# vwxyzjn/cleanrl

Measured on NVIDIA H100. Metric: env steps/sec (SPS) PPO Breakout num_envs=1024, higher is better.
Workload: dtype bf16

## Files before the change

### cleanrl_b200/csrc/net_tc.cu

```cuda
#include <cuda.h>
#include <algorithm>
#include "tc_base.cuh"
#include "tc_conv_win.cuh"
#include "tc_conv23.cuh"
#include "tc_conv1_u8.cuh"
#include "tc_gemm_tma.cuh"
#include "tc_wgrad_win.cuh"
#include "tc_reduce.cuh"
#include "tc_aux.cuh"
#include "tc_heads.cuh"
#include "tc_heads_wide.cuh"
#include "tc_lstm.cuh"

namespace b200rl {

struct NatureLayout {
    int A;
    int64_t c1w, c1b, c2w, c2b, c3w, c3b, fcw, fcb, hw, hb, total;
    int64_t w1f, w2f, w2dg, w3f, w3dg, wfcf, wfcdg, w1l, w1sc, packed_total;
    bool wide; int G; int64_t whf, whdg, hbp;
    int64_t wih, whh, bih, bhh, whhp;
    explicit NatureLayout(int A_) : A(A_), wih(-1), whh(-1), bih(-1), bhh(-1), whhp(-1) {
        int64_t o = 0;
        c1w = o; o += 32 * 4 * 8 * 8;  c1b = o; o += 32;
// ... 83 lines not shown
    p.A = x; p.M = n; p.nchunks = nchunks;
}


static void win_defaults(WinParams& p) { memset(&p, 0, sizeof(p)); p.scale = 1.f; }
static int round8(int v) { return (v + 7) & ~7; }
static void win_conv1(WinParams& p, const bf16* x0, const int64_t* rows, int64_t n) {
    p.A = x0; p.rows = rows; p.n = (int)n; p.G = 441; p.Wp = 21; p.M = n * 441;
    p.tpi_shift = 2;
    p.n_images = rows ? (int64_t)1 << 24 : n;
    p.ntaps = 4; p.shift[0] = 0; p.shift[1] = 1; p.shift[2] = 21; p.shift[3] = 22; p.WR = round8(128 + 22);
}
static void wgw_defaults(WGradWinParams& w) { memset(&w, 0, sizeof(w)); }

static const int kC1Ctas = 264, kC2Ctas = 132, kC3Ctas = 132;
static WPlan conv1_wgrad_plan(int64_t n, bool u8) {
    return u8 ? wgrad_plan(n * 512, kC2Ctas, 512) : wgrad_plan(n * 512, kC1Ctas, 128);
}
static WPlan conv2_wgrad_plan(int64_t n) { return wgrad_plan(n * 100, kC2Ctas, 128); }
static WPlan conv3_wgrad_plan(int64_t n) { return wgrad_plan(n * 81, kC3Ctas, 128); }

static size_t wgrad_win_bytes(int splits, int nslots) { return (size_t)splits * nslots * 64 * 64 * sizeof(float); }
static size_t wgrad_win_bias_bytes(int splits) { return (size_t)splits * 64 * sizeof(float); }
static int launch_wgrad_win(const WGradWinParams& p, int ctas, cudaStream_t s, const char* what) {
    const size_t smem = (size_t)kWgradWinStages * ((size_t)p.WRX * 128 * p.cpr + 128 * 128) + 4096 + 1024;
    static SmemAttrCache attr;
    if (int rc0 = attr.ensure(tc_wgrad_win, smem, what)) return rc0;
    CUtensorMap tmX, tmY;
    memset(&tmX, 0, sizeof(tmX)); memset(&tmY, 0, sizeof(tmY));
    const int use_tma = p.tpi_shift ? 0 : 1;
    if (p.rows_per_cta % 128 != 0) return fail(B200RL_ERR_INVALID_ARGUMENT, "%s: rows per CTA must be a multiple of 128", what);
    if (ctas < 1 || (int64_t)(ctas - 1) * p.rows_per_cta >= p.M)
        return fail(B200RL_ERR_INVALID_ARGUMENT, "%s: every row split must own at least one row", what);
    int rc;
    if (use_tma) {
        if (p.rows || p.ldy != 64 || p.ncolsY != 64)
            return fail(B200RL_ERR_INVALID_ARGUMENT, "%s: linear-grid mode needs contiguous rows and 64-channel dY", what);
        if ((rc = make_tmap_2d(&tmX, p.X, p.M, (int64_t)p.cpr * 64, p.WRX, what))) return rc;
        if ((rc = make_tmap_2d(&tmY, p.Y, p.M, 64, 128, what))) return rc;
    } else {
        if ((128 << p.tpi_shift) < p.G) return fail(B200RL_ERR_INVALID_ARGUMENT, "%s: steps per image too small", what);
        if ((rc = make_tmap_3d(&tmX, p.X, p.n_images, p.G, (int64_t)p.cpr * 64, p.WRX, what))) return rc;
    }
    const dim3 grid((unsigned)ceil_div(p.nslots / 2, kWgradWinTilesPerCta), ctas);
    tc_wgrad_win<<<grid, kWgradWinThreads, smem, s>>>(tmX, tmY, p, use_tma);
    return check_launch(what);
}

}

using namespace b200rl;

namespace b200rl {
static bool head_ok(int A) { return A >= 1 && A < kMaxWideHeads; }
static size_t wide_dhead_bytes(int64_t n, const NatureLayout& L) { return ((size_t)n * L.G * 2 + 255) & ~(size_t)255; }
static size_t wide_small_bytes(int64_t n, const NatureLayout& L, int A1) {
    return wide_dhead_bytes(n, L) + colsum_f32_ws(n, A1);
}

static int trunk_fwd(const NatureLayout& L, const NatureActs& Q, const float* params, const bf16* P, bf16* act, int64_t n,
                     cudaStream_t s) {
    int rc;
    KGemmParams p;
    Conv23Params cp;
    cp.n = (int)n; cp.b2 = params + L.c2b; cp.b3 = params + L.c3b; cp.act2 = act + Q.act2; cp.act3 = act + Q.act3;
    cp.m2 = reinterpret_cast<uint32_t*>(act + Q.m2); cp.m3 = reinterpret_cast<uint32_t*>(act + Q.m3);
    { ProfScope ps(s, "conv23_fwd", 2.0 * n * 81 * 64 * 512 + 2.0 * n * 49 * 64 * 576,
                   (double)n * (12800 * 2 + 5184 * 2 + 648 + 3136 * 2 + 392));
// ... 8 lines not shown
}

static int trunk_bwd(const NatureLayout& L, const NatureActs& Q, const bf16* P, bf16* act, float* grads, int64_t n,
                     float* wsbig, float* wssmall, void* tail_ready_event, bool dact1_fused, cudaStream_t s) {
    int rc;
    KGemmParams p;
    {
        int splits;
        { ProfScope ps(s, "fc_wgrad", 2.0 * n * 512 * 3136, (double)n * (3136 + 512) * 2 + 512.0 * 3136 * 4);
          if ((splits = launch_wgrad_tma(act + Q.dhid, 512, act + Q.act3, 3136, n, wsbig, s, "naturecnn/fc_wgrad")) < 0) return splits; }
        { ProfScope ps(s, "wgrad_fold_bias", 0, 0);
          note_launches(1); tc_fold_fc<<<(unsigned)ceil_div((int64_t)512 * 3136, 256), 256, 0, s>>>(wsbig, splits, 512, 13 * 256, 512, 3136, 64, 49, 1.f, grads + L.fcw);
          if ((rc = colsum(act + Q.dhid, n, 512, 512, wssmall, grads + L.fcb, s))) return rc; }
        if (tail_ready_event) {
            cudaError_t e = cudaEventRecord(reinterpret_cast<cudaEvent_t>(tail_ready_event), s);
            if (e != cudaSuccess) return fail(B200RL_ERR_CUDA, "naturecnn_backward: cudaEventRecord: %s", cudaGetErrorString(e));
        }
        gemm_rowmajor(p, act + Q.dhid, n, 8);
        p.Bw = P + L.wfcdg; p.N = 3136; p.out = act + Q.dact3a; p.out2 = act + Q.dact3b; p.dual_dact3 = 1;
        p.ldo = 3136; p.mask_bits = reinterpret_cast<const uint32_t*>(act + Q.m3);
        { ProfScope ps(s, "fc_dgrad", 2.0 * n * 512 * 3136, (double)n * ((3136 + 512) * 2 + 392) + 512.0 * 3136 * 2);
          if ((rc = launch_gemm_tma<128, 3>(p, s, "naturecnn/fc_dgrad"))) return rc; }
    }
    WGradWinParams gw;
    WinParams wp;
    FoldWin fw;
    {
        wgw_defaults(gw);
        gw.X = act + Q.act2; gw.M = n * 81; gw.n = (int)n; gw.G = 81; gw.cpr = 1; gw.nslots = 10; gw.WRX = round8(128 + 20);
        for (int t = 0; t < 9; ++t) gw.shift[t] = (t / 3) * 9 + (t % 3);
        const int st[10] = {0, 1, 2, 3, 4, 5, 6, 7, 7, 8};
        for (int k = 0; k < 10; ++k) { gw.slot_tap[k] = st[k]; gw.slot_cc[k] = 0; }
        gw.Y = act + Q.dact3a; gw.ldy = 64; gw.ncolsY = 64;
        const WPlan pl = conv3_wgrad_plan(n);
        gw.rows_per_cta = pl.rows_per_cta; gw.ws = wsbig; gw.wsb = wssmall;
        { ProfScope ps(s, "conv3_wgrad", 2.0 * n * 49 * 64 * 576, (double)n * (5184 + 5184) * 2);
          if ((rc = launch_wgrad_win(gw, pl.splits, s, "naturecnn/conv3_wgrad"))) return rc; }
        memset(&fw, 0, sizeof(fw));
        fw.layer = 3; fw.S = pl.splits; fw.nslots = 10; fw.Cout = 64; fw.scale = 1.f; fw.bscale = 1.f;
        for (int k = 0; k < 10; ++k) { fw.slot_tap[k] = st[k]; fw.slot_skip[k] = (k == 8); }
        { ProfScope ps(s, "wgrad_fold_bias", 0, 0);
          fw.wsb = wssmall; fw.db = grads + L.c3b;
          tc_fold_win<<<(unsigned)ceil_div(640 * 64 + 64, 32), 256, 0, s>>>(wsbig, fw, grads + L.c3w);
          if ((rc = check_launch("naturecnn/conv3_fold"))) return rc; }
        win_defaults(wp);
        wp.A = act + Q.dact3b; wp.n = (int)n; wp.G = 121; wp.Wp = 11; wp.M = n * 121; wp.ntaps = 9;
        for (int ky = 0; ky < 3; ++ky) for (int kx = 0; kx < 3; ++kx) wp.shift[ky * 3 + kx] = (2 - ky) * 11 + (2 - kx);
        wp.WR = round8(128 + 24);
        wp.Bw = P + L.w3dg; wp.N = 64; wp.vH = 9; wp.vW = 9; wp.out_mode = WOUT_DACT2;
        wp.out = act + Q.dact2a; wp.out2 = act + Q.dact2b; wp.mask_bits = reinterpret_cast<const uint32_t*>(act + Q.m2);
        { ProfScope ps(s, "conv3_dgrad", 2.0 * n * 81 * 64 * 576, (double)n * ((7744 + 6400 + 7744) * 2 + 648));
          if ((rc = launch_conv_win_t<128, 1, 4, 9>(wp, s, "naturecnn/conv3_dgrad"))) return rc; }
    }
    {
        wgw_defaults(gw);
        gw.X = act + Q.act1; gw.M = n * 100; gw.n = (int)n; gw.G = 100; gw.cpr = 2; gw.nslots = 8; gw.WRX = round8(128 + 11);
        gw.shift[0] = 0; gw.shift[1] = 1; gw.shift[2] = 10; gw.shift[3] = 11;
        for (int k = 0; k < 8; ++k) { gw.slot_tap[k] = k >> 1; gw.slot_cc[k] = k & 1; }
        gw.Y = act + Q.dact2a; gw.ldy = 64; gw.ncolsY = 64;
        const WPlan pl = conv2_wgrad_plan(n);
        gw.rows_per_cta = pl.rows_per_cta; gw.ws = wsbig; gw.wsb = wssmall;
        { ProfScope ps(s, "conv2_wgrad", 2.0 * n * 81 * 64 * 512, (double)n * (12800 + 6400) * 2);
          if ((rc = launch_wgrad_win(gw, pl.splits, s, "naturecnn/conv2_wgrad"))) return rc; }
        memset(&fw, 0, sizeof(fw));
        fw.layer = 2; fw.S = pl.splits; fw.nslots = 8; fw.Cout = 64; fw.scale = 1.f; fw.bscale = 1.f;
        for (int k = 0; k < 8; ++k) { fw.slot_tap[k] = k >> 1; fw.slot_cc[k] = k & 1; }
        { ProfScope ps(s, "wgrad_fold_bias", 0, 0);
          fw.wsb = wssmall; fw.db = grads + L.c2b;
          tc_fold_win<<<(unsigned)ceil_div(512 * 64 + 64, 32), 256, 0, s>>>(wsbig, fw, grads + L.c2w);
          if ((rc = check_launch("naturecnn/conv2_fold"))) return rc; }
        if (dact1_fused) return B200RL_OK;
        win_defaults(wp);
        wp.A = act + Q.dact2b; wp.n = (int)n; wp.G = 121; wp.Wp = 11; wp.M = n * 121; wp.ntaps = 4;
        for (int a = 0; a < 2; ++a) for (int b = 0; b < 2; ++b) wp.shift[a * 2 + b] = (1 - a) * 11 + (1 - b);
        wp.WR = round8(128 + 12);
        wp.Bw = P + L.w2dg; wp.N = 128; wp.vH = 10; wp.vW = 10; wp.out_mode = WOUT_DACT1;
        wp.out = act + Q.dact1; wp.mask_bits = reinterpret_cast<const uint32_t*>(act + Q.m1);
        { ProfScope ps(s, "conv2_dgrad", 2.0 * n * 400 * 32 * 256, (double)n * ((7744 + 14112) * 2 + 1600));
          if ((rc = launch_conv_win<128, 1, 4, 4>(wp, s, "naturecnn/conv2_dgrad"))) return rc; }
    }
    return B200RL_OK;
}
static size_t trunk_big_bytes(int64_t n) {
    return std::max({wgrad_tma_bytes(n, 512, 3136), wgrad_win_bytes(conv3_wgrad_plan(n).splits, 10),
                     wgrad_win_bytes(conv2_wgrad_plan(n).splits, 8)});
}
// ... 422 lines not shown
```

### cleanrl_b200/csrc/tc_reduce.cuh

```cuda
#pragma once
#include "tc_base.cuh"
#include "tc_wgrad_win.cuh"

namespace b200rl {
using namespace tc;

__device__ __forceinline__ float zlane_sum(const float* __restrict__ part, int64_t slab, int nslabs, int64_t idx, bool valid,
                                           float* red ) {
    const int zl = threadIdx.x >> 5, ol = threadIdx.x & 31;
    float s = 0.f;
    if (valid) {
        int z = zl;
        for (; z + 24 < nslabs; z += 32) {
            const float v0 = part[(int64_t)z * slab + idx], v1 = part[(int64_t)(z + 8) * slab + idx];
            const float v2 = part[(int64_t)(z + 16) * slab + idx], v3 = part[(int64_t)(z + 24) * slab + idx];
            s += v0; s += v1; s += v2; s += v3;
        }
        for (; z < nslabs; z += 8) s += part[(int64_t)z * slab + idx];
    }
    red[threadIdx.x] = s;
    __syncthreads();
    float t = 0.f;
    if (zl == 0) {
#pragma unroll
        for (int l = 0; l < 8; ++l) t += red[l * 32 + ol];
    }
    return t;
}

struct FoldWin { int layer, S, nslots, Cout; int slot_tap[16], slot_cc[16], slot_skip[16]; float scale;
                 float bscale;
                 const float* wsb; float* db; };
static __global__ void __launch_bounds__(256) tc_fold_win(const float* __restrict__ ws, const FoldWin f, float* __restrict__ dst) {
    __shared__ float red[256];
    const int idx = blockIdx.x * 32 + (threadIdx.x & 31);
    const int KX = f.nslots * 64;
    if (idx >= KX * f.Cout) {
        const int co = idx - KX * f.Cout;
        const bool valid = co < f.Cout && f.db != nullptr;
        const float s = zlane_sum(f.wsb, 64, f.S, co, valid, red);
        if (valid && threadIdx.x < 32) f.db[co] = s * f.bscale;
        return;
    }
    const int xi = idx / f.Cout, co = idx - xi * f.Cout;
    const int slot = xi >> 6, row = xi & 63;
    const bool valid = !f.slot_skip[slot];
    float s = zlane_sum(ws, (int64_t)KX * 64, f.S, (int64_t)xi * 64 + co, valid, red);
    if (!valid || threadIdx.x >= 32) return;
    s *= f.scale;
    const int tap = f.slot_tap[slot];
    int64_t o;
    if (f.layer == 1) {
        const int c = row >> 4, sy = (row >> 2) & 3, sx = row & 3;
        o = (((int64_t)co * 4 + c) * 8 + ((tap >> 1) * 4 + sy)) * 8 + (tap & 1) * 4 + sx;
    } else if (f.layer == 2) {
        const int q = f.slot_cc[slot] * 64 + row;
        const int g = q >> 5, c = q & 31;
        o = (((int64_t)co * 32 + c) * 4 + (2 * (tap >> 1) + (g >> 1))) * 4 + 2 * (tap & 1) + (g & 1);
    } else {
        o = ((int64_t)co * 64 + row) * 9 + tap;
    }
    dst[o] = s;
}

static __global__ void tc_fold_fc(const float* __restrict__ ws, int S, int KX, int NY, int validX, int validY,
                           int C, int KK, float scale, float* __restrict__ dst) {
    const int64_t idx = (int64_t)blockIdx.x * blockDim.x + threadIdx.x;
    const int64_t total = (int64_t)validX * validY;
    if (idx >= total) return;
    const int xi = (int)(idx / validY), yi = (int)(idx - (int64_t)xi * validY);
    float s = 0.f;
// ... 62 lines not shown
```

### cleanrl_b200/csrc/tc_wgmma.cuh

```cuda
#pragma once
#include <cstdint>

namespace b200rl { namespace tc {

__device__ __forceinline__ void wgmma_fence() { asm volatile("wgmma.fence.sync.aligned;" ::: "memory"); }
__device__ __forceinline__ void wgmma_commit() { asm volatile("wgmma.commit_group.sync.aligned;" ::: "memory"); }
template <int N>
__device__ __forceinline__ void wgmma_wait() { asm volatile("wgmma.wait_group.sync.aligned %0;" ::"n"(N) : "memory"); }
template <class T, int R>
__device__ __forceinline__ void wgmma_fence_operands(T (&d)[R]) {
#pragma unroll
    for (int i = 0; i < R; ++i) asm volatile("" : "+r"(reinterpret_cast<uint32_t&>(d[i]))::"memory");
}

template <int N, int TA, int TB> struct WgmmaBf16;
template <int TA, int TB> struct WgmmaBf16<32, TA, TB> {
    __device__ __forceinline__ static void mma(float (&d)[16], uint64_t adesc, uint64_t bdesc, uint32_t accumulate) {
        asm volatile(
            "{\n\t.reg .pred p;\n\tsetp.ne.b32 p, %18, 0;\n\t"
            "wgmma.mma_async.sync.aligned.m64n32k16.f32.bf16.bf16 {"
            "%0, %1, %2, %3, %4, %5, %6, %7, %8, %9, %10, %11, %12, %13, %14, %15"
            "}, %16, %17, p, 1, 1, %19, %20;\n\t}\n"
            : "+f"(d[0]), "+f"(d[1]), "+f"(d[2]), "+f"(d[3]), "+f"(d[4]), "+f"(d[5]), "+f"(d[6]), "+f"(d[7]),
              "+f"(d[8]), "+f"(d[9]), "+f"(d[10]), "+f"(d[11]), "+f"(d[12]), "+f"(d[13]), "+f"(d[14]), "+f"(d[15])
// ... 34 lines not shown
    }
};
template <int TA, int TB> struct WgmmaBf16<128, TA, TB> {
    __device__ __forceinline__ static void mma(float (&d)[64], uint64_t adesc, uint64_t bdesc, uint32_t accumulate) {
        asm volatile(
            "{\n\t.reg .pred p;\n\tsetp.ne.b32 p, %66, 0;\n\t"
            "wgmma.mma_async.sync.aligned.m64n128k16.f32.bf16.bf16 {"
            "%0, %1, %2, %3, %4, %5, %6, %7, %8, %9, %10, %11, %12, %13, %14, %15, "
            "%16, %17, %18, %19, %20, %21, %22, %23, %24, %25, %26, %27, %28, %29, %30, %31, "
            "%32, %33, %34, %35, %36, %37, %38, %39, %40, %41, %42, %43, %44, %45, %46, %47, "
            "%48, %49, %50, %51, %52, %53, %54, %55, %56, %57, %58, %59, %60, %61, %62, %63"
            "}, %64, %65, p, 1, 1, %67, %68;\n\t}\n"
            : "+f"(d[0]), "+f"(d[1]), "+f"(d[2]), "+f"(d[3]), "+f"(d[4]), "+f"(d[5]), "+f"(d[6]), "+f"(d[7]),
              "+f"(d[8]), "+f"(d[9]), "+f"(d[10]), "+f"(d[11]), "+f"(d[12]), "+f"(d[13]), "+f"(d[14]), "+f"(d[15]),
              "+f"(d[16]), "+f"(d[17]), "+f"(d[18]), "+f"(d[19]), "+f"(d[20]), "+f"(d[21]), "+f"(d[22]), "+f"(d[23]),
              "+f"(d[24]), "+f"(d[25]), "+f"(d[26]), "+f"(d[27]), "+f"(d[28]), "+f"(d[29]), "+f"(d[30]), "+f"(d[31]),
              "+f"(d[32]), "+f"(d[33]), "+f"(d[34]), "+f"(d[35]), "+f"(d[36]), "+f"(d[37]), "+f"(d[38]), "+f"(d[39]),
              "+f"(d[40]), "+f"(d[41]), "+f"(d[42]), "+f"(d[43]), "+f"(d[44]), "+f"(d[45]), "+f"(d[46]), "+f"(d[47]),
              "+f"(d[48]), "+f"(d[49]), "+f"(d[50]), "+f"(d[51]), "+f"(d[52]), "+f"(d[53]), "+f"(d[54]), "+f"(d[55]),
              "+f"(d[56]), "+f"(d[57]), "+f"(d[58]), "+f"(d[59]), "+f"(d[60]), "+f"(d[61]), "+f"(d[62]), "+f"(d[63])
            : "l"(adesc), "l"(bdesc), "r"(accumulate), "n"(TA), "n"(TB));
    }
};
template <int TA, int TB> struct WgmmaBf16<256, TA, TB> {
    __device__ __forceinline__ static void mma(float (&d)[128], uint64_t adesc, uint64_t bdesc, uint32_t accumulate) {
        asm volatile(
            "{\n\t.reg .pred p;\n\tsetp.ne.b32 p, %130, 0;\n\t"
            "wgmma.mma_async.sync.aligned.m64n256k16.f32.bf16.bf16 {"
            "%0, %1, %2, %3, %4, %5, %6, %7, %8, %9, %10, %11, %12, %13, %14, %15, "
            "%16, %17, %18, %19, %20, %21, %22, %23, %24, %25, %26, %27, %28, %29, %30, %31, "
            "%32, %33, %34, %35, %36, %37, %38, %39, %40, %41, %42, %43, %44, %45, %46, %47, "
            "%48, %49, %50, %51, %52, %53, %54, %55, %56, %57, %58, %59, %60, %61, %62, %63, "
            "%64, %65, %66, %67, %68, %69, %70, %71, %72, %73, %74, %75, %76, %77, %78, %79, "
            "%80, %81, %82, %83, %84, %85, %86, %87, %88, %89, %90, %91, %92, %93, %94, %95, "
            "%96, %97, %98, %99, %100, %101, %102, %103, %104, %105, %106, %107, %108, %109, %110, %111, "
            "%112, %113, %114, %115, %116, %117, %118, %119, %120, %121, %122, %123, %124, %125, %126, %127"
            "}, %128, %129, p, 1, 1, %131, %132;\n\t}\n"
            : "+f"(d[0]), "+f"(d[1]), "+f"(d[2]), "+f"(d[3]), "+f"(d[4]), "+f"(d[5]), "+f"(d[6]), "+f"(d[7]),
              "+f"(d[8]), "+f"(d[9]), "+f"(d[10]), "+f"(d[11]), "+f"(d[12]), "+f"(d[13]), "+f"(d[14]), "+f"(d[15]),
              "+f"(d[16]), "+f"(d[17]), "+f"(d[18]), "+f"(d[19]), "+f"(d[20]), "+f"(d[21]), "+f"(d[22]), "+f"(d[23]),
              "+f"(d[24]), "+f"(d[25]), "+f"(d[26]), "+f"(d[27]), "+f"(d[28]), "+f"(d[29]), "+f"(d[30]), "+f"(d[31]),
              "+f"(d[32]), "+f"(d[33]), "+f"(d[34]), "+f"(d[35]), "+f"(d[36]), "+f"(d[37]), "+f"(d[38]), "+f"(d[39]),
              "+f"(d[40]), "+f"(d[41]), "+f"(d[42]), "+f"(d[43]), "+f"(d[44]), "+f"(d[45]), "+f"(d[46]), "+f"(d[47]),
              "+f"(d[48]), "+f"(d[49]), "+f"(d[50]), "+f"(d[51]), "+f"(d[52]), "+f"(d[53]), "+f"(d[54]), "+f"(d[55]),
              "+f"(d[56]), "+f"(d[57]), "+f"(d[58]), "+f"(d[59]), "+f"(d[60]), "+f"(d[61]), "+f"(d[62]), "+f"(d[63]),
              "+f"(d[64]), "+f"(d[65]), "+f"(d[66]), "+f"(d[67]), "+f"(d[68]), "+f"(d[69]), "+f"(d[70]), "+f"(d[71]),
// ... 41 lines not shown
```

### cleanrl_b200/csrc/tc_wgrad_win.cuh

```cuda
#pragma once
#include "tc_base.cuh"

namespace b200rl {
using namespace tc;

constexpr int kWgradWinStages = 3;
struct WGradWinParams {
    const bf16* X; const int64_t* rows; int64_t M; int n, G;
    int tpi_shift;
    int64_t n_images;
    int cpr;
    int nslots;
    int slot_tap[16], slot_cc[16];
    int shift[16];
    int WRX;
    const bf16* Y; int ldy, ncolsY;
    int64_t rows_per_cta;
    float* ws;
    float* wsb;
};

constexpr int kWgradWinThreads = 512;
constexpr int kWgradWinTilesPerCta = 2;

template <int NT>
__device__ __forceinline__ void wgrad_win_mma(const WGradWinParams& p, uint8_t* smem, int stage_bytes, int XBYTES, int IMGX,
                                              uint64_t* full_bar, uint64_t* empty_bar, int nsteps, int t0, int w, int tid) {
    constexpr int R = 128, STAGES = kWgradWinStages, NY = 64;
    const int wt = tid & 127;
    uint32_t arel[NT];
#pragma unroll
    for (int tt = 0; tt < NT; ++tt) {
        const int slot = 2 * (t0 + tt) + w;
        arel[tt] = (uint32_t)(p.slot_cc[slot] * IMGX + p.shift[p.slot_tap[slot]] * 128);
    }
    float d[NT][NY / 2];
#pragma unroll
    for (int tt = 0; tt < NT; ++tt)
#pragma unroll
        for (int e = 0; e < NY / 2; ++e) d[tt][e] = 0.f;
    auto step = [&](int it) {
        const int s = it % STAGES;
        mbar_wait(&full_bar[s], (it / STAGES) & 1);
        wgmma_fence();
        const uint32_t xa = smem_u32(smem + (size_t)s * stage_bytes), ya = xa + XBYTES;
        const uint64_t yd = desc_mnmajor(ya, 0);
#pragma unroll
        for (int tt = 0; tt < NT; ++tt) {
            const uint64_t xd = desc_mnmajor(xa + arel[tt], 0);
#pragma unroll
            for (int kk = 0; kk < R / 16; ++kk)
                WgmmaBf16<NY, 1, 1>::mma(d[tt], xd + kk * 128, yd + kk * 128, (it | kk) != 0 ? 1u : 0u);
        }
        wgmma_commit();
    };
    for (int it = 0; it + 1 < nsteps; ++it) {
        step(it);
        wgmma_wait<1>();
        if (it > 0 && (tid & 31) == 0) mbar_arrive(&empty_bar[(it - 1) % STAGES]);
    }
    step(nsteps - 1);
    wgmma_wait<0>();
    const int row = ((wt >> 5) << 4) + ((wt & 31) >> 2), col = (wt & 3) * 2;
    float* wsb = p.ws + (int64_t)blockIdx.y * (p.nslots * 64) * NY;
#pragma unroll
    for (int tt = 0; tt < NT; ++tt) {
        wgmma_fence_operands(d[tt]);
        float* d0 = wsb + (int64_t)((2 * (t0 + tt) + w) * 64 + row) * NY + col;
#pragma unroll
        for (int j = 0; j < NY / 8; ++j) {
            *reinterpret_cast<float2*>(d0 + 8 * j) = make_float2(d[tt][4 * j], d[tt][4 * j + 1]);
            *reinterpret_cast<float2*>(d0 + 8 * NY + 8 * j) = make_float2(d[tt][4 * j + 2], d[tt][4 * j + 3]);
        }
    }
}

static __global__ void __launch_bounds__(kWgradWinThreads, 1) tc_wgrad_win(const __grid_constant__ CUtensorMap tmX, const __grid_constant__ CUtensorMap tmY,
                                                       const WGradWinParams p, int use_tma) {
    constexpr int R = 128, STAGES = kWgradWinStages, LOOKAHEAD = 1, NY = 64, TT = kWgradWinTilesPerCta;
    static_assert(TT == 2, "the wgmma warpgroups dispatch on 1 or 2 tiles per CTA");
    extern __shared__ uint8_t smem_raw[];
    __shared__ uint64_t full_bar[STAGES], empty_bar[STAGES];
    uint8_t* smem = reinterpret_cast<uint8_t*>((reinterpret_cast<uintptr_t>(smem_raw) + 1023) & ~uintptr_t(1023));
    const int tid = threadIdx.x, warp = tid >> 5;
    const int IMGX = p.WRX * 128;
    const int XBYTES = IMGX * p.cpr;
    const int stage_bytes = XBYTES + R * 128;
    const int xt = p.nslots / 2;
    const int t0 = blockIdx.x * TT;
    float* sRed = reinterpret_cast<float*>(smem + (size_t)STAGES * stage_bytes);
    if (tid == 0) {
        for (int s = 0; s < STAGES; ++s) { mbar_init(&full_bar[s], use_tma ? 1 : 5); mbar_init(&empty_bar[s], (use_tma ? 4 : 0) + 8); }
        fence_barrier_init();
        tma_prefetch_desc(&tmX);
        if (use_tma) tma_prefetch_desc(&tmY);
    }
    __syncthreads();
    const int64_t m_begin = (int64_t)blockIdx.y * p.rows_per_cta;
    int64_t m_end = m_begin + p.rows_per_cta;
    if (m_end > p.M) m_end = p.M;
    const int nsteps = m_end > m_begin ? (int)((m_end - m_begin + R - 1) / R) : 0;
    const int tmask = (1 << p.tpi_shift) - 1;
    const int64_t g0 = m_begin / R;

    if (warp == 4) {
        if ((tid & 31) == 0) {
            int z_next = 0;
            if (!use_tma && nsteps > 0) {
                const int64_t img = g0 >> p.tpi_shift;
                z_next = p.rows ? (int)__ldg(p.rows + (img < p.n ? img : 0)) : (int)img;
            }
            for (int it = 0; it < nsteps; ++it) {
                const int s = it % STAGES;
                const int z = z_next;
                if (!use_tma && it + 1 < nsteps) {
                    const int64_t img1 = (g0 + it + 1) >> p.tpi_shift;
                    z_next = p.rows ? (int)__ldg(p.rows + (img1 < p.n ? img1 : 0)) : (int)img1;
                }
                if (it >= STAGES) mbar_wait(&empty_bar[s], ((it / STAGES) - 1) & 1);
                const uint32_t dst = smem_u32(smem + (size_t)s * stage_bytes);
                if (use_tma) {
                    const int m0 = (int)(m_begin + (int64_t)it * R);
                    mbar_arrive_expect_tx(&full_bar[s], (uint32_t)stage_bytes);
                    for (int c = 0; c < p.cpr; ++c) tma_load_2d(dst + c * IMGX, &tmX, c * 64, m0, &full_bar[s]);
                    tma_load_2d(dst + XBYTES, &tmY, 0, m0, &full_bar[s]);
                } else {
                    const int t_in = (int)((g0 + it) & tmask);
                    mbar_arrive_expect_tx(&full_bar[s], (uint32_t)XBYTES);
                    for (int c = 0; c < p.cpr; ++c) tma_load_3d(dst + c * IMGX, &tmX, c * 64, t_in * 128, z, &full_bar[s]);
                }
            }
        }
    } else if (warp < 4) {
        const int rq = tid >> 3, c16 = tid & 7;
        float bsum[8];
#pragma unroll
        for (int e = 0; e < 8; ++e) bsum[e] = 0.f;
        auto add_step = [&](const uint8_t* sYp) {
#pragma unroll
            for (int ps = 0; ps < R / 16; ++ps) {
                const int rr = ps * 16 + rq;
                const int4 v = *reinterpret_cast<const int4*>(sYp + img_off(rr, c16));
                const uint32_t w[4] = {(uint32_t)v.x, (uint32_t)v.y, (uint32_t)v.z, (uint32_t)v.w};
#pragma unroll
                for (int e = 0; e < 4; ++e) {
                    bsum[2 * e] += __uint_as_float(w[e] << 16);
                    bsum[2 * e + 1] += __uint_as_float(w[e] & 0xFFFF0000u);
                }
            }
        };
        if (use_tma) {
            for (int it = 0; it < nsteps; ++it) {
                const int s = it % STAGES;
                mbar_wait(&full_bar[s], (it / STAGES) & 1);
                add_step(smem + (size_t)s * stage_bytes + XBYTES);
                __syncwarp();
                if ((tid & 31) == 0) mbar_arrive(&empty_bar[s]);
            }
        } else {
            for (int it = 0; it < nsteps; ++it) {
                const int s = it % STAGES;
                const int64_t g = g0 + it;
                const int64_t img = g >> p.tpi_shift;
                const int t_in = (int)(g & tmask);
                if (it >= STAGES) mbar_wait(&empty_bar[s], ((it / STAGES) - 1) & 1);
                const uint32_t sY = smem_u32(smem + (size_t)s * stage_bytes + XBYTES);
#pragma unroll
                for (int ps = 0; ps < R / 16; ++ps) {
                    const int rr = ps * 16 + rq;
                    const int rl = t_in * 128 + rr;
                    const int col = c16 * 8;
                    const bool ok = rl < p.G && img < p.n && col < p.ncolsY;
                    cp_async16(sY + img_off(rr, c16), p.Y + (ok ? (img * p.G + rl) * (int64_t)p.ldy + col : 0), ok ? 16u : 0u);
                }
                cp_async_commit();
                if (it >= LOOKAHEAD) {
                    cp_async_wait<LOOKAHEAD>();
                    const int sd = (it - LOOKAHEAD) % STAGES;
                    add_step(smem + (size_t)sd * stage_bytes + XBYTES);
                    fence_proxy_async_smem();
                    __syncwarp();
                    if ((tid & 31) == 0) mbar_arrive(&full_bar[sd]);
                }
            }
            cp_async_wait<0>();
            for (int d = (nsteps >= LOOKAHEAD ? nsteps - LOOKAHEAD : 0); d < nsteps; ++d)
                add_step(smem + (size_t)(d % STAGES) * stage_bytes + XBYTES);
            fence_proxy_async_smem();
            __syncwarp();
            if ((tid & 31) == 0)
                for (int d = (nsteps >= LOOKAHEAD ? nsteps - LOOKAHEAD : 0); d < nsteps; ++d) mbar_arrive(&full_bar[d % STAGES]);
        }
#pragma unroll
        for (int e = 0; e < 8; ++e) sRed[rq * 64 + c16 * 8 + e] = bsum[e];
        asm volatile("bar.sync 1, 128;" ::: "memory");
        if (tid < 64) {
            float t = 0.f;
#pragma unroll
            for (int l = 0; l < 16; ++l) t += sRed[l * 64 + tid];
            if (blockIdx.x == 0) p.wsb[(int64_t)blockIdx.y * NY + tid] = t;
        }
    } else if (warp >= 8) {
        const int w = (warp - 8) >> 2;
        if (xt - t0 >= TT) wgrad_win_mma<TT>(p, smem, stage_bytes, XBYTES, IMGX, full_bar, empty_bar, nsteps, t0, w, tid);
        else wgrad_win_mma<1>(p, smem, stage_bytes, XBYTES, IMGX, full_bar, empty_bar, nsteps, t0, w, tid);
    }
}

}
```

Baseline: 1.313 million.

## Replace conv2/conv3 weight-gradient window kernel with row-tap wide-N wgmma kernel

Adds a templated tc_wgrad_rows kernel that computes conv2 and conv3 weight gradients by treating dY as the A operand and shifted input windows as a wide N operand (n192/n128 wgmma). Several kernel taps along a row are covered by one wgmma. This replaces the old per-slot-pair tiling, whose grid was split over slot tiles and reloaded the same data for each, and it drops the padded duplicate slot for conv3. The new kernel uses a 4-stage TMA pipeline that loads both X and dY, and folds the bias reduction into the producer warpgroup. The old window kernel is simplified to a single 2-tile, 3D-TMA path. The trade-off is large per-thread accumulator arrays and a transposed scattered store into the workspace.

```diff
diff --git a/cleanrl_b200/csrc/net_tc.cu b/cleanrl_b200/csrc/net_tc.cu
--- a/cleanrl_b200/csrc/net_tc.cu
+++ b/cleanrl_b200/csrc/net_tc.cu
@@ -129,28 +129,41 @@
 
 static size_t wgrad_win_bytes(int splits, int nslots) { return (size_t)splits * nslots * 64 * 64 * sizeof(float); }
 static size_t wgrad_win_bias_bytes(int splits) { return (size_t)splits * 64 * sizeof(float); }
+static int check_splits(int64_t M, int64_t rows_per_cta, int ctas, const char* what) {
+    if (rows_per_cta % 128 != 0) return fail(B200RL_ERR_INVALID_ARGUMENT, "%s: rows per CTA must be a multiple of 128", what);
+    if (ctas < 1 || (int64_t)(ctas - 1) * rows_per_cta >= M)
+        return fail(B200RL_ERR_INVALID_ARGUMENT, "%s: every row split must own at least one row", what);
+    return B200RL_OK;
+}
 static int launch_wgrad_win(const WGradWinParams& p, int ctas, cudaStream_t s, const char* what) {
     const size_t smem = (size_t)kWgradWinStages * ((size_t)p.WRX * 128 * p.cpr + 128 * 128) + 4096 + 1024;
     static SmemAttrCache attr;
-    if (int rc0 = attr.ensure(tc_wgrad_win, smem, what)) return rc0;
+    int rc;
+    if ((rc = attr.ensure(tc_wgrad_win, smem, what))) return rc;
+    if ((rc = check_splits(p.M, p.rows_per_cta, ctas, what))) return rc;
+    if (p.nslots != 4) return fail(B200RL_ERR_INVALID_ARGUMENT, "%s: the wgmma warpgroups take 2 output tiles of 2 slots", what);
+    if ((128 << p.tpi_shift) < p.G) return fail(B200RL_ERR_INVALID_ARGUMENT, "%s: steps per image too small", what);
+    CUtensorMap tmX;
+    memset(&tmX, 0, sizeof(tmX));
+    if ((rc = make_tmap_3d(&tmX, p.X, p.n_images, p.G, (int64_t)p.cpr * 64, p.WRX, what))) return rc;
+    tc_wgrad_win<<<ctas, kWgradWinThreads, smem, s>>>(tmX, p);
+    return check_launch(what);
+}
+template <int CPR, int KROWS, int TPR, int WP, int NCW>
+static int launch_wgrad_rows(const bf16* X, const bf16* Y, int64_t M, const WPlan& pl, float* ws, float* wsb, cudaStream_t s,
+                             const char* what) {
+    using C = WgradRowsCfg<CPR, KROWS, TPR, WP, NCW>;
+    static SmemAttrCache attr;
+    int rc;
+    if ((rc = attr.ensure(tc_wgrad_rows<CPR, KROWS, TPR, WP, NCW>, C::kSmem, what))) return rc;
+    if ((rc = check_splits(M, pl.rows_per_cta, pl.splits, what))) return rc;
     CUtensorMap tmX, tmY;
     memset(&tmX, 0, sizeof(tmX)); memset(&tmY, 0, sizeof(tmY));
-    const int use_tma = p.tpi_shift ? 0 : 1;
-    if (p.rows_per_cta % 128 != 0) return fail(B200RL_ERR_INVALID_ARGUMENT, "%s: rows per CTA must be a multiple of 128", what);
-    if (ctas < 1 || (int64_t)(ctas - 1) * p.rows_per_cta >= p.M)
-        return fail(B200RL_ERR_INVALID_ARGUMENT, "%s: every row split must own at least one row", what);
-    int rc;
-    if (use_tma) {
-        if (p.rows || p.ldy != 64 || p.ncolsY != 64)
-            return fail(B200RL_ERR_INVALID_ARGUMENT, "%s: linear-grid mode needs contiguous rows and 64-channel dY", what);
-        if ((rc = make_tmap_2d(&tmX, p.X, p.M, (int64_t)p.cpr * 64, p.WRX, what))) return rc;
-        if ((rc = make_tmap_2d(&tmY, p.Y, p.M, 64, 128, what))) return rc;
-    } else {
-        if ((128 << p.tpi_shift) < p.G) return fail(B200RL_ERR_INVALID_ARGUMENT, "%s: steps per image too small", what);
-        if ((rc = make_tmap_3d(&tmX, p.X, p.n_images, p.G, (int64_t)p.cpr * 64, p.WRX, what))) return rc;
-    }
-    const dim3 grid((unsigned)ceil_div(p.nslots / 2, kWgradWinTilesPerCta), ctas);
-    tc_wgrad_win<<<grid, kWgradWinThreads, smem, s>>>(tmX, tmY, p, use_tma);
+    if ((rc = make_tmap_2d(&tmX, X, M, (int64_t)CPR * 64, C::kWRX, what))) return rc;
+    if ((rc = make_tmap_2d(&tmY, Y, M, 64, 128, what))) return rc;
+    WGradRowsParams p;
+    p.M = M; p.rows_per_cta = pl.rows_per_cta; p.ws = ws; p.wsb = wsb;
+    tc_wgrad_rows<CPR, KROWS, TPR, WP, NCW><<<pl.splits, C::kThreads, C::kSmem, s>>>(tmX, tmY, p);
     return check_launch(what);
 }
 
@@ -205,26 +218,19 @@
         { ProfScope ps(s, "fc_dgrad", 2.0 * n * 512 * 3136, (double)n * ((3136 + 512) * 2 + 392) + 512.0 * 3136 * 2);
           if ((rc = launch_gemm_tma<128, 3>(p, s, "naturecnn/fc_dgrad"))) return rc; }
     }
-    WGradWinParams gw;
     WinParams wp;
     FoldWin fw;
     {
-        wgw_defaults(gw);
-        gw.X = act + Q.act2; gw.M = n * 81; gw.n = (int)n; gw.G = 81; gw.cpr = 1; gw.nslots = 10; gw.WRX = round8(128 + 20);
-        for (int t = 0; t < 9; ++t) gw.shift[t] = (t / 3) * 9 + (t % 3);
-        const int st[10] = {0, 1, 2, 3, 4, 5, 6, 7, 7, 8};
-        for (int k = 0; k < 10; ++k) { gw.slot_tap[k] = st[k]; gw.slot_cc[k] = 0; }
-        gw.Y = act + Q.dact3a; gw.ldy = 64; gw.ncolsY = 64;
         const WPlan pl = conv3_wgrad_plan(n);
-        gw.rows_per_cta = pl.rows_per_cta; gw.ws = wsbig; gw.wsb = wssmall;
         { ProfScope ps(s, "conv3_wgrad", 2.0 * n * 49 * 64 * 576, (double)n * (5184 + 5184) * 2);
-          if ((rc = launch_wgrad_win(gw, pl.splits, s, "naturecnn/conv3_wgrad"))) return rc; }
+          if ((rc = launch_wgrad_rows<1, 3, 3, 9, 3>(act + Q.act2, act + Q.dact3a, n * 81, pl, wsbig, wssmall, s,
+                                                      "naturecnn/conv3_wgrad"))) return rc; }
         memset(&fw, 0, sizeof(fw));
-        fw.layer = 3; fw.S = pl.splits; fw.nslots = 10; fw.Cout = 64; fw.scale = 1.f; fw.bscale = 1.f;
-        for (int k = 0; k < 10; ++k) { fw.slot_tap[k] = st[k]; fw.slot_skip[k] = (k == 8); }
+        fw.layer = 3; fw.S = pl.splits; fw.nslots = 9; fw.Cout = 64; fw.scale = 1.f; fw.bscale = 1.f;
+        for (int k = 0; k < 9; ++k) fw.slot_tap[k] = k;
         { ProfScope ps(s, "wgrad_fold_bias", 0, 0);
           fw.wsb = wssmall; fw.db = grads + L.c3b;
-          tc_fold_win<<<(unsigned)ceil_div(640 * 64 + 64, 32), 256, 0, s>>>(wsbig, fw, grads + L.c3w);
+          tc_fold_win<<<(unsigned)ceil_div(576 * 64 + 64, 32), 256, 0, s>>>(wsbig, fw, grads + L.c3w);
           if ((rc = check_launch("naturecnn/conv3_fold"))) return rc; }
         win_defaults(wp);
         wp.A = act + Q.dact3b; wp.n = (int)n; wp.G = 121; wp.Wp = 11; wp.M = n * 121; wp.ntaps = 9;
@@ -236,15 +242,10 @@
           if ((rc = launch_conv_win_t<128, 1, 4, 9>(wp, s, "naturecnn/conv3_dgrad"))) return rc; }
     }
     {
-        wgw_defaults(gw);
-        gw.X = act + Q.act1; gw.M = n * 100; gw.n = (int)n; gw.G = 100; gw.cpr = 2; gw.nslots = 8; gw.WRX = round8(128 + 11);
-        gw.shift[0] = 0; gw.shift[1] = 1; gw.shift[2] = 10; gw.shift[3] = 11;
-        for (int k = 0; k < 8; ++k) { gw.slot_tap[k] = k >> 1; gw.slot_cc[k] = k & 1; }
-        gw.Y = act + Q.dact2a; gw.ldy = 64; gw.ncolsY = 64;
         const WPlan pl = conv2_wgrad_plan(n);
-        gw.rows_per_cta = pl.rows_per_cta; gw.ws = wsbig; gw.wsb = wssmall;
         { ProfScope ps(s, "conv2_wgrad", 2.0 * n * 81 * 64 * 512, (double)n * (12800 + 6400) * 2);
-          if ((rc = launch_wgrad_win(gw, pl.splits, s, "naturecnn/conv2_wgrad"))) return rc; }
+          if ((rc = launch_wgrad_rows<2, 2, 2, 10, 2>(act + Q.act1, act + Q.dact2a, n * 100, pl, wsbig, wssmall, s,
+                                                       "naturecnn/conv2_wgrad"))) return rc; }
         memset(&fw, 0, sizeof(fw));
         fw.layer = 2; fw.S = pl.splits; fw.nslots = 8; fw.Cout = 64; fw.scale = 1.f; fw.bscale = 1.f;
         for (int k = 0; k < 8; ++k) { fw.slot_tap[k] = k >> 1; fw.slot_cc[k] = k & 1; }
diff --git a/cleanrl_b200/csrc/tc_reduce.cuh b/cleanrl_b200/csrc/tc_reduce.cuh
--- a/cleanrl_b200/csrc/tc_reduce.cuh
+++ b/cleanrl_b200/csrc/tc_reduce.cuh
@@ -28,7 +28,7 @@
     return t;
 }
 
-struct FoldWin { int layer, S, nslots, Cout; int slot_tap[16], slot_cc[16], slot_skip[16]; float scale;
+struct FoldWin { int layer, S, nslots, Cout; int slot_tap[16], slot_cc[16]; float scale;
                  float bscale;
                  const float* wsb; float* db; };
 static __global__ void __launch_bounds__(256) tc_fold_win(const float* __restrict__ ws, const FoldWin f, float* __restrict__ dst) {
@@ -44,9 +44,8 @@
     }
     const int xi = idx / f.Cout, co = idx - xi * f.Cout;
     const int slot = xi >> 6, row = xi & 63;
-    const bool valid = !f.slot_skip[slot];
-    float s = zlane_sum(ws, (int64_t)KX * 64, f.S, (int64_t)xi * 64 + co, valid, red);
-    if (!valid || threadIdx.x >= 32) return;
+    float s = zlane_sum(ws, (int64_t)KX * 64, f.S, (int64_t)xi * 64 + co, true, red);
+    if (threadIdx.x >= 32) return;
     s *= f.scale;
     const int tap = f.slot_tap[slot];
     int64_t o;
diff --git a/cleanrl_b200/csrc/tc_wgmma.cuh b/cleanrl_b200/csrc/tc_wgmma.cuh
--- a/cleanrl_b200/csrc/tc_wgmma.cuh
+++ b/cleanrl_b200/csrc/tc_wgmma.cuh
@@ -80,6 +80,33 @@
             : "l"(adesc), "l"(bdesc), "r"(accumulate), "n"(TA), "n"(TB));
     }
 };
+template <int TA, int TB> struct WgmmaBf16<192, TA, TB> {
+    __device__ __forceinline__ static void mma(float (&d)[96], uint64_t adesc, uint64_t bdesc, uint32_t accumulate) {
+        asm volatile(
+            "{\n\t.reg .pred p;\n\tsetp.ne.b32 p, %98, 0;\n\t"
+            "wgmma.mma_async.sync.aligned.m64n192k16.f32.bf16.bf16 {"
+            "%0, %1, %2, %3, %4, %5, %6, %7, %8, %9, %10, %11, %12, %13, %14, %15, "
+            "%16, %17, %18, %19, %20, %21, %22, %23, %24, %25, %26, %27, %28, %29, %30, %31, "
+            "%32, %33, %34, %35, %36, %37, %38, %39, %40, %41, %42, %43, %44, %45, %46, %47, "
+            "%48, %49, %50, %51, %52, %53, %54, %55, %56, %57, %58, %59, %60, %61, %62, %63, "
+            "%64, %65, %66, %67, %68, %69, %70, %71, %72, %73, %74, %75, %76, %77, %78, %79, "
+            "%80, %81, %82, %83, %84, %85, %86, %87, %88, %89, %90, %91, %92, %93, %94, %95"
+            "}, %96, %97, p, 1, 1, %99, %100;\n\t}\n"
+            : "+f"(d[0]), "+f"(d[1]), "+f"(d[2]), "+f"(d[3]), "+f"(d[4]), "+f"(d[5]), "+f"(d[6]), "+f"(d[7]),
+              "+f"(d[8]), "+f"(d[9]), "+f"(d[10]), "+f"(d[11]), "+f"(d[12]), "+f"(d[13]), "+f"(d[14]), "+f"(d[15]),
+              "+f"(d[16]), "+f"(d[17]), "+f"(d[18]), "+f"(d[19]), "+f"(d[20]), "+f"(d[21]), "+f"(d[22]), "+f"(d[23]),
+              "+f"(d[24]), "+f"(d[25]), "+f"(d[26]), "+f"(d[27]), "+f"(d[28]), "+f"(d[29]), "+f"(d[30]), "+f"(d[31]),
+              "+f"(d[32]), "+f"(d[33]), "+f"(d[34]), "+f"(d[35]), "+f"(d[36]), "+f"(d[37]), "+f"(d[38]), "+f"(d[39]),
+              "+f"(d[40]), "+f"(d[41]), "+f"(d[42]), "+f"(d[43]), "+f"(d[44]), "+f"(d[45]), "+f"(d[46]), "+f"(d[47]),
+              "+f"(d[48]), "+f"(d[49]), "+f"(d[50]), "+f"(d[51]), "+f"(d[52]), "+f"(d[53]), "+f"(d[54]), "+f"(d[55]),
+              "+f"(d[56]), "+f"(d[57]), "+f"(d[58]), "+f"(d[59]), "+f"(d[60]), "+f"(d[61]), "+f"(d[62]), "+f"(d[63]),
+              "+f"(d[64]), "+f"(d[65]), "+f"(d[66]), "+f"(d[67]), "+f"(d[68]), "+f"(d[69]), "+f"(d[70]), "+f"(d[71]),
+              "+f"(d[72]), "+f"(d[73]), "+f"(d[74]), "+f"(d[75]), "+f"(d[76]), "+f"(d[77]), "+f"(d[78]), "+f"(d[79]),
+              "+f"(d[80]), "+f"(d[81]), "+f"(d[82]), "+f"(d[83]), "+f"(d[84]), "+f"(d[85]), "+f"(d[86]), "+f"(d[87]),
+              "+f"(d[88]), "+f"(d[89]), "+f"(d[90]), "+f"(d[91]), "+f"(d[92]), "+f"(d[93]), "+f"(d[94]), "+f"(d[95])
+            : "l"(adesc), "l"(bdesc), "r"(accumulate), "n"(TA), "n"(TB));
+    }
+};
 template <int TA, int TB> struct WgmmaBf16<256, TA, TB> {
     __device__ __forceinline__ static void mma(float (&d)[128], uint64_t adesc, uint64_t bdesc, uint32_t accumulate) {
         asm volatile(
diff --git a/cleanrl_b200/csrc/tc_wgrad_win.cuh b/cleanrl_b200/csrc/tc_wgrad_win.cuh
--- a/cleanrl_b200/csrc/tc_wgrad_win.cuh
+++ b/cleanrl_b200/csrc/tc_wgrad_win.cuh
@@ -3,6 +3,33 @@
 
 namespace b200rl {
 using namespace tc;
+
+__device__ __forceinline__ void wgrad_bias_add_step(float (&bsum)[8], const uint8_t* sYp, int tid) {
+    const int rq = tid >> 3, c16 = tid & 7;
+#pragma unroll
+    for (int ps = 0; ps < 128 / 16; ++ps) {
+        const int rr = ps * 16 + rq;
+        const int4 v = *reinterpret_cast<const int4*>(sYp + img_off(rr, c16));
+        const uint32_t w[4] = {(uint32_t)v.x, (uint32_t)v.y, (uint32_t)v.z, (uint32_t)v.w};
+#pragma unroll
+        for (int e = 0; e < 4; ++e) {
+            bsum[2 * e] += __uint_as_float(w[e] << 16);
+            bsum[2 * e + 1] += __uint_as_float(w[e] & 0xFFFF0000u);
+        }
+    }
+}
+__device__ __forceinline__ void wgrad_bias_store(const float (&bsum)[8], float* sRed , float* wsb, int tid) {
+    const int rq = tid >> 3, c16 = tid & 7;
+#pragma unroll
+    for (int e = 0; e < 8; ++e) sRed[rq * 64 + c16 * 8 + e] = bsum[e];
+    asm volatile("bar.sync 1, 128;" ::: "memory");
+    if (tid < 64) {
+        float t = 0.f;
+#pragma unroll
+        for (int l = 0; l < 16; ++l) t += sRed[l * 64 + tid];
+        wsb[tid] = t;
+    }
+}
 
 constexpr int kWgradWinStages = 3;
 struct WGradWinParams {
@@ -21,17 +48,16 @@
 };
 
 constexpr int kWgradWinThreads = 512;
-constexpr int kWgradWinTilesPerCta = 2;
 
 template <int NT>
 __device__ __forceinline__ void wgrad_win_mma(const WGradWinParams& p, uint8_t* smem, int stage_bytes, int XBYTES, int IMGX,
-                                              uint64_t* full_bar, uint64_t* empty_bar, int nsteps, int t0, int w, int tid) {
+                                              uint64_t* full_bar, uint64_t* empty_bar, int nsteps, int w, int tid) {
     constexpr int R = 128, STAGES = kWgradWinStages, NY = 64;
     const int wt = tid & 127;
     uint32_t arel[NT];
 #pragma unroll
     for (int tt = 0; tt < NT; ++tt) {
-        const int slot = 2 * (t0 + tt) + w;
+        const int slot = 2 * tt + w;
         arel[tt] = (uint32_t)(p.slot_cc[slot] * IMGX + p.shift[p.slot_tap[slot]] * 128);
     }
     float d[NT][NY / 2];
@@ -62,11 +88,11 @@
     step(nsteps - 1);
     wgmma_wait<0>();
     const int row = ((wt >> 5) << 4) + ((wt & 31) >> 2), col = (wt & 3) * 2;
-    float* wsb = p.ws + (int64_t)blockIdx.y * (p.nslots * 64) * NY;
+    float* wsb = p.ws + (int64_t)blockIdx.x * (p.nslots * 64) * NY;
 #pragma unroll
     for (int tt = 0; tt < NT; ++tt) {
         wgmma_fence_operands(d[tt]);
-        float* d0 = wsb + (int64_t)((2 * (t0 + tt) + w) * 64 + row) * NY + col;
+        float* d0 = wsb + (int64_t)((2 * tt + w) * 64 + row) * NY + col;
 #pragma unroll
         for (int j = 0; j < NY / 8; ++j) {
             *reinterpret_cast<float2*>(d0 + 8 * j) = make_float2(d[tt][4 * j], d[tt][4 * j + 1]);
@@ -75,10 +101,8 @@
     }
 }
 
-static __global__ void __launch_bounds__(kWgradWinThreads, 1) tc_wgrad_win(const __grid_constant__ CUtensorMap tmX, const __grid_constant__ CUtensorMap tmY,
-                                                       const WGradWinParams p, int use_tma) {
-    constexpr int R = 128, STAGES = kWgradWinStages, LOOKAHEAD = 1, NY = 64, TT = kWgradWinTilesPerCta;
-    static_assert(TT == 2, "the wgmma warpgroups dispatch on 1 or 2 tiles per CTA");
+static __global__ void __launch_bounds__(kWgradWinThreads, 1) tc_wgrad_win(const __grid_constant__ CUtensorMap tmX, const WGradWinParams p) {
+    constexpr int R = 128, STAGES = kWgradWinStages, LOOKAHEAD = 1;
     extern __shared__ uint8_t smem_raw[];
     __shared__ uint64_t full_bar[STAGES], empty_bar[STAGES];
     uint8_t* smem = reinterpret_cast<uint8_t*>((reinterpret_cast<uintptr_t>(smem_raw) + 1023) & ~uintptr_t(1023));
@@ -86,17 +110,14 @@
     const int IMGX = p.WRX * 128;
     const int XBYTES = IMGX * p.cpr;
     const int stage_bytes = XBYTES + R * 128;
-    const int xt = p.nslots / 2;
-    const int t0 = blockIdx.x * TT;
     float* sRed = reinterpret_cast<float*>(smem + (size_t)STAGES * stage_bytes);
     if (tid == 0) {
-        for (int s = 0; s < STAGES; ++s) { mbar_init(&full_bar[s], use_tma ? 1 : 5); mbar_init(&empty_bar[s], (use_tma ? 4 : 0) + 8); }
+        for (int s = 0; s < STAGES; ++s) { mbar_init(&full_bar[s], 5); mbar_init(&empty_bar[s], 8); }
         fence_barrier_init();
         tma_prefetch_desc(&tmX);
-        if (use_tma) tma_prefetch_desc(&tmY);
     }
     __syncthreads();
-    const int64_t m_begin = (int64_t)blockIdx.y * p.rows_per_cta;
+    const int64_t m_begin = (int64_t)blockIdx.x * p.rows_per_cta;
     int64_t m_end = m_begin + p.rows_per_cta;
     if (m_end > p.M) m_end = p.M;
     const int nsteps = m_end > m_begin ? (int)((m_end - m_begin + R - 1) / R) : 0;
@@ -106,29 +127,22 @@
     if (warp == 4) {
         if ((tid & 31) == 0) {
             int z_next = 0;
-            if (!use_tma && nsteps > 0) {
+            if (nsteps > 0) {
                 const int64_t img = g0 >> p.tpi_shift;
                 z_next = p.rows ? (int)__ldg(p.rows + (img < p.n ? img : 0)) : (int)img;
             }
             for (int it = 0; it < nsteps; ++it) {
                 const int s = it % STAGES;
                 const int z = z_next;
-                if (!use_tma && it + 1 < nsteps) {
+                if (it + 1 < nsteps) {
                     const int64_t img1 = (g0 + it + 1) >> p.tpi_shift;
                     z_next = p.rows ? (int)__ldg(p.rows + (img1 < p.n ? img1 : 0)) : (int)img1;
                 }
                 if (it >= STAGES) mbar_wait(&empty_bar[s], ((it / STAGES) - 1) & 1);
                 const uint32_t dst = smem_u32(smem + (size_t)s * stage_bytes);
-                if (use_tma) {
-                    const int m0 = (int)(m_begin + (int64_t)it * R);
-                    mbar_arrive_expect_tx(&full_bar[s], (uint32_t)stage_bytes);
-                    for (int c = 0; c < p.cpr; ++c) tma_load_2d(dst + c * IMGX, &tmX, c * 64, m0, &full_bar[s]);
-                    tma_load_2d(dst + XBYTES, &tmY, 0, m0, &full_bar[s]);
-                } else {
-                    const int t_in = (int)((g0 + it) & tmask);
-                    mbar_arrive_expect_tx(&full_bar[s], (uint32_t)XBYTES);
-                    for (int c = 0; c < p.cpr; ++c) tma_load_3d(dst + c * IMGX, &tmX, c * 64, t_in * 128, z, &full_bar[s]);
-                }
+                const int t_in = (int)((g0 + it) & tmask);
+                mbar_arrive_expect_tx(&full_bar[s], (uint32_t)XBYTES);
+                for (int c = 0; c < p.cpr; ++c) tma_load_3d(dst + c * IMGX, &tmX, c * 64, t_in * 128, z, &full_bar[s]);
             }
         }
     } else if (warp < 4) {
@@ -136,75 +150,158 @@
         float bsum[8];
 #pragma unroll
         for (int e = 0; e < 8; ++e) bsum[e] = 0.f;
-        auto add_step = [&](const uint8_t* sYp) {
+        for (int it = 0; it < nsteps; ++it) {
+            const int s = it % STAGES;
+            const int64_t g = g0 + it;
+            const int64_t img = g >> p.tpi_shift;
+            const int t_in = (int)(g & tmask);
+            if (it >= STAGES) mbar_wait(&empty_bar[s], ((it / STAGES) - 1) & 1);
+            const uint32_t sY = smem_u32(smem + (size_t)s * stage_bytes + XBYTES);
 #pragma unroll
             for (int ps = 0; ps < R / 16; ++ps) {
                 const int rr = ps * 16 + rq;
-                const int4 v = *reinterpret_cast<const int4*>(sYp + img_off(rr, c16));
-                const uint32_t w[4] = {(uint32_t)v.x, (uint32_t)v.y, (uint32_t)v.z, (uint32_t)v.w};
-#pragma unroll
-                for (int e = 0; e < 4; ++e) {
-                    bsum[2 * e] += __uint_as_float(w[e] << 16);
-                    bsum[2 * e + 1] += __uint_as_float(w[e] & 0xFFFF0000u);
-                }
-            }
+                const int rl = t_in * 128 + rr;
+                const int col = c16 * 8;
+                const bool ok = rl < p.G && img < p.n && col < p.ncolsY;
+                cp_async16(sY + img_off(rr, c16), p.Y + (ok ? (img * p.G + rl) * (int64_t)p.ldy + col : 0), ok ? 16u : 0u);
+            }
+            cp_async_commit();
+            if (it >= LOOKAHEAD) {
+                cp_async_wait<LOOKAHEAD>();
+                const int sd = (it - LOOKAHEAD) % STAGES;
+                wgrad_bias_add_step(bsum, smem + (size_t)sd * stage_bytes + XBYTES, tid);
+                fence_proxy_async_smem();
+                __syncwarp();
+                if ((tid & 31) == 0) mbar_arrive(&full_bar[sd]);
+            }
+        }
+        cp_async_wait<0>();
+        for (int d = (nsteps >= LOOKAHEAD ? nsteps - LOOKAHEAD : 0); d < nsteps; ++d)
+            wgrad_bias_add_step(bsum, smem + (size_t)(d % STAGES) * stage_bytes + XBYTES, tid);
+        fence_proxy_async_smem();
+        __syncwarp();
+        if ((tid & 31) == 0)
+            for (int d = (nsteps >= LOOKAHEAD ? nsteps - LOOKAHEAD : 0); d < nsteps; ++d) mbar_arrive(&full_bar[d % STAGES]);
+        wgrad_bias_store(bsum, sRed, p.wsb + (int64_t)blockIdx.x * 64, tid);
+    } else if (warp >= 8) {
+        wgrad_win_mma<2>(p, smem, stage_bytes, XBYTES, IMGX, full_bar, empty_bar, nsteps, (warp - 8) >> 2, tid);
+    }
+}
+
+constexpr int kWgradRowsStages = 4;
+struct WGradRowsParams {
+    int64_t M;
+    int64_t rows_per_cta;
+    float* ws;
+    float* wsb;
+};
+template <int CPR, int KROWS, int TPR, int WP, int NCW>
+struct WgradRowsCfg {
+    static constexpr int kUnits = KROWS * CPR, kUnitsPerWg = kUnits / NCW, kN = 64 * TPR;
+    static constexpr int kSlots = KROWS * TPR * CPR;
+    static constexpr int kThreads = 128 + 128 * NCW;
+    static constexpr int kWRX = (128 + (KROWS - 1) * WP + TPR - 1 + 7) & ~7;
+    static constexpr int kImgX = kWRX * 128, kXBytes = kImgX * CPR, kStageBytes = kXBytes + 128 * 128;
+    static constexpr size_t kSmem = (size_t)kWgradRowsStages * kStageBytes + 4096 + 1024;
+    static_assert(kUnits % NCW == 0, "every wgmma warpgroup owns the same number of units");
+    static_assert(kUnitsPerWg * kN / 2 + 24 <= ((65536 / kThreads) & ~7), "accumulators exceed the registers of a thread");
+    static_assert(kSmem <= 227 * 1024, "stages exceed shared memory");
+};
+
+template <int CPR, int KROWS, int TPR, int WP, int NCW>
+static __global__ void __launch_bounds__(WgradRowsCfg<CPR, KROWS, TPR, WP, NCW>::kThreads, 1)
+tc_wgrad_rows(const __grid_constant__ CUtensorMap tmX, const __grid_constant__ CUtensorMap tmY, const WGradRowsParams p) {
+    using C = WgradRowsCfg<CPR, KROWS, TPR, WP, NCW>;
+    constexpr int R = 128, STAGES = kWgradRowsStages, U = C::kUnitsPerWg, NACC = C::kN / 2;
+    extern __shared__ uint8_t smem_raw[];
+    __shared__ uint64_t full_bar[STAGES], empty_bar[STAGES];
+    uint8_t* smem = reinterpret_cast<uint8_t*>((reinterpret_cast<uintptr_t>(smem_raw) + 1023) & ~uintptr_t(1023));
+    const int tid = threadIdx.x, warp = tid >> 5;
+    float* sRed = reinterpret_cast<float*>(smem + (size_t)STAGES * C::kStageBytes);
+    if (tid == 0) {
+        for (int s = 0; s < STAGES; ++s) { mbar_init(&full_bar[s], 1); mbar_init(&empty_bar[s], 4 + 4 * NCW); }
+        fence_barrier_init();
+        tma_prefetch_desc(&tmX);
+        tma_prefetch_desc(&tmY);
+    }
+    __syncthreads();
+    const int64_t m_begin = (int64_t)blockIdx.x * p.rows_per_cta;
+    int64_t m_end = m_begin + p.rows_per_cta;
+    if (m_end > p.M) m_end = p.M;
+    const int nsteps = (int)((m_end - m_begin + R - 1) / R);
+
+    if (warp < 4) {
+        auto issue = [&](int j) {
+            const int s = j % STAGES;
+            if (j >= STAGES) mbar_wait(&empty_bar[s], ((j / STAGES) - 1) & 1);
+            const uint32_t dst = smem_u32(smem + (size_t)s * C::kStageBytes);
+            const int m0 = (int)(m_begin + (int64_t)j * R);
+            mbar_arrive_expect_tx(&full_bar[s], (uint32_t)C::kStageBytes);
+#pragma unroll
+            for (int c = 0; c < CPR; ++c) tma_load_2d(dst + c * C::kImgX, &tmX, c * 64, m0, &full_bar[s]);
+            tma_load_2d(dst + C::kXBytes, &tmY, 0, m0, &full_bar[s]);
         };
-        if (use_tma) {
-            for (int it = 0; it < nsteps; ++it) {
-                const int s = it % STAGES;
-                mbar_wait(&full_bar[s], (it / STAGES) & 1);
-                add_step(smem + (size_t)s * stage_bytes + XBYTES);
-                __syncwarp();
-                if ((tid & 31) == 0) mbar_arrive(&empty_bar[s]);
-            }
-        } else {
-            for (int it = 0; it < nsteps; ++it) {
-                const int s = it % STAGES;
-                const int64_t g = g0 + it;
-                const int64_t img = g >> p.tpi_shift;
-                const int t_in = (int)(g & tmask);
-                if (it >= STAGES) mbar_wait(&empty_bar[s], ((it / STAGES) - 1) & 1);
-                const uint32_t sY = smem_u32(smem + (size_t)s * stage_bytes + XBYTES);
-#pragma unroll
-                for (int ps = 0; ps < R / 16; ++ps) {
-                    const int rr = ps * 16 + rq;
-                    const int rl = t_in * 128 + rr;
-                    const int col = c16 * 8;
-                    const bool ok = rl < p.G && img < p.n && col < p.ncolsY;
-                    cp_async16(sY + img_off(rr, c16), p.Y + (ok ? (img * p.G + rl) * (int64_t)p.ldy + col : 0), ok ? 16u : 0u);
-                }
-                cp_async_commit();
-                if (it >= LOOKAHEAD) {
-                    cp_async_wait<LOOKAHEAD>();
-                    const int sd = (it - LOOKAHEAD) % STAGES;
-                    add_step(smem + (size_t)sd * stage_bytes + XBYTES);
-                    fence_proxy_async_smem();
-                    __syncwarp();
-                    if ((tid & 31) == 0) mbar_arrive(&full_bar[sd]);
-                }
-            }
-            cp_async_wait<0>();
-            for (int d = (nsteps >= LOOKAHEAD ? nsteps - LOOKAHEAD : 0); d < nsteps; ++d)
-                add_step(smem + (size_t)(d % STAGES) * stage_bytes + XBYTES);
-            fence_proxy_async_smem();
+        if (tid == 0)
+            for (int j = 0; j < STAGES - 1 && j < nsteps; ++j) issue(j);
+        float bsum[8];
+#pragma unroll
+        for (int e = 0; e < 8; ++e) bsum[e] = 0.f;
+        for (int it = 0; it < nsteps; ++it) {
+            if (tid == 0 && it + STAGES - 1 < nsteps) issue(it + STAGES - 1);
+            const int s = it % STAGES;
+            mbar_wait(&full_bar[s], (it / STAGES) & 1);
+            wgrad_bias_add_step(bsum, smem + (size_t)s * C::kStageBytes + C::kXBytes, tid);
             __syncwarp();
-            if ((tid & 31) == 0)
-                for (int d = (nsteps >= LOOKAHEAD ? nsteps - LOOKAHEAD : 0); d < nsteps; ++d) mbar_arrive(&full_bar[d % STAGES]);
-        }
-#pragma unroll
-        for (int e = 0; e < 8; ++e) sRed[rq * 64 + c16 * 8 + e] = bsum[e];
-        asm volatile("bar.sync 1, 128;" ::: "memory");
-        if (tid < 64) {
-            float t = 0.f;
-#pragma unroll
-            for (int l = 0; l < 16; ++l) t += sRed[l * 64 + tid];
-            if (blockIdx.x == 0) p.wsb[(int64_t)blockIdx.y * NY + tid] = t;
-        }
-    } else if (warp >= 8) {
-        const int w = (warp - 8) >> 2;
-        if (xt - t0 >= TT) wgrad_win_mma<TT>(p, smem, stage_bytes, XBYTES, IMGX, full_bar, empty_bar, nsteps, t0, w, tid);
-        else wgrad_win_mma<1>(p, smem, stage_bytes, XBYTES, IMGX, full_bar, empty_bar, nsteps, t0, w, tid);
-    }
-}
-
-}
+            if ((tid & 31) == 0) mbar_arrive(&empty_bar[s]);
+        }
+        wgrad_bias_store(bsum, sRed, p.wsb + (int64_t)blockIdx.x * 64, tid);
+    } else {
+        const int w = (warp >> 2) - 1, wt = tid & 127;
+        float d[U][NACC];
+#pragma unroll
+        for (int uu = 0; uu < U; ++uu)
+#pragma unroll
+            for (int e = 0; e < NACC; ++e) d[uu][e] = 0.f;
+        auto brel = [&](int uu) { const int u = w * U + uu; return (uint32_t)((u % CPR) * C::kImgX + (u / CPR) * WP * 128); };
+        auto step = [&](int it) {
+            const int s = it % STAGES;
+            mbar_wait(&full_bar[s], (it / STAGES) & 1);
+            wgmma_fence();
+            const uint32_t xa = smem_u32(smem + (size_t)s * C::kStageBytes), ya = xa + C::kXBytes;
+            const uint64_t yd = desc_mnmajor(ya, 0);
+#pragma unroll
+            for (int uu = 0; uu < U; ++uu) {
+                const uint64_t xd = desc_mnmajor(xa + brel(uu), 128);
+#pragma unroll
+                for (int kk = 0; kk < R / 16; ++kk)
+                    WgmmaBf16<C::kN, 1, 1>::mma(d[uu], yd + kk * 128, xd + kk * 128, (it | kk) != 0 ? 1u : 0u);
+            }
+            wgmma_commit();
+        };
+        for (int it = 0; it + 1 < nsteps; ++it) {
+            step(it);
+            wgmma_wait<1>();
+            if (it > 0 && (tid & 31) == 0) mbar_arrive(&empty_bar[(it - 1) % STAGES]);
+        }
+        step(nsteps - 1);
+        wgmma_wait<0>();
+        const int co = ((wt >> 5) << 4) + ((wt & 31) >> 2), col = (wt & 3) * 2;
+        float* wsp = p.ws + (int64_t)blockIdx.x * (C::kSlots * 64 * 64);
+#pragma unroll
+        for (int uu = 0; uu < U; ++uu) {
+            wgmma_fence_operands(d[uu]);
+            const int u = w * U + uu;
+#pragma unroll
+            for (int j = 0; j < NACC / 4; ++j) {
+                const int slot = ((u / CPR) * TPR + (j >> 3)) * CPR + u % CPR;
+                float* q = wsp + (int64_t)(slot * 64 + (8 * j & 63) + col) * 64 + co;
+                q[0] = d[uu][4 * j];
+                q[64] = d[uu][4 * j + 1];
+                q[8] = d[uu][4 * j + 2];
+                q[64 + 8] = d[uu][4 * j + 3];
+            }
+        }
+    }
+}
+
+}
```

Result: faster. 1.359 million (median of 6 runs) (+3.5%).
